# willow-ahrens/ChainPartitioners.jl

Measured on AMD Instinct MI355X. Metric: partitions/sec, DynamicTotalSplitter(AffineConnectivityModel{Int64}(0,0,0,1)), K=64, higher is better.
Workload: dtype int64; 1 GPU; config 3: DynamicTotalSplitter(AffineConnectivityModel{Int64}(0,0,0,1)) on suitesparse_shaped CSR (seeded SplitMix64 generator, tests/synth.py), n=10000000 rows, nnz=100000000, K=64; one independent partition per GPU; n=10000000, nnz=100000000, K=64, includes_oracle_build=True, device_block_pool=True

## Files before the change

### chainpartitioners.jl_amd/_lib.py

```python
from __future__ import annotations

import ctypes as C
import os
from functools import partial
import weakref

import numpy as np

from . import models as M

_HERE = os.path.dirname(os.path.abspath(__file__))
LIB_PATH = os.environ.get("CP_LIB_PATH") or os.path.join(_HERE, "libchainpart.so")


class _Array:

    def __init__(self, dtype, name):
        self.dtype, self.name, self.what = np.dtype(dtype), name, np.dtype(dtype).name

    def _accepts(self, a):
        return a.dtype == self.dtype

    def from_param(self, a):
        if a is None:
# ... 76 lines not shown
    "cp_dp_ptr_at": (_i32, [_vp, _i64, _i64, _pi64]),
    "cp_dp_ptr_row": (_i32, [_vp, _i64, _I64("out")]),
    "cp_dp_set_window": (_i32, [_vp, _i64]),
    "cp_dp_set_rows": (_i32, [_vp, _i64, _i64]),
    "cp_dp_block_tables": (_i32, [_vp, _pi32, _I64("opt_out"), _I64("nets_out"), _I64("selfnets_out")]),
    "cp_dp_destroy": (_i32, [_vp]),
    "cp_set_stream": (_i32, [_vp, _vp]),
    "cp_reset_stream": (_i32, [_vp]),
    "cp_get_stat": (_i32, [_str, _pi64]),
    "cp_test_round_scans": (_i32, [_I32("a"), _i64, _i64, _I32("b"), _i64, _i64, _i32, _i64, _i64, _i32, _i32,
                                   _I64("offs_out"), _I64("toffs_out"), _I64("res")]),
    "cp_test_fix_merge": (_i32, [_MODEL, _i64, _I64("toffs"), _I64("part_v"), _I32("part_p"), _I32("part_nn"), _I32("part_nl"), _I32("tile_s"),
                                 _I32("tile_s2"), _I32("anchor"), _I32("anchor2"), _I32("row"), _I32("plane"), _i64, _i32, _I32("p_out"),
                                 _I32("nn_out"), _I32("nl_out"), _I64("res")]),
    "cp_test_own_split": (_i32, [_vp, _I32("vpos_out"), _I32("vsa_out"), _I32("vnext_out"), _I64("res")]),
    "cp_set_option": (_i32, [_str, _i64]),
    "cp_prof_enable": (_i32, [_i32]),
    "cp_prof_reset": (_i32, []),
    "cp_prof_get": (_i32, [_i32, C.POINTER(C.c_char_p), _pi64, _pf64, _pf64]),
}
SYMBOLS = list(SIGNATURES)

_lib = None


def _typed(name, fn, restype, argtypes):
    fn.restype, fn.argtypes = restype, argtypes

    def call(*args):
        try:
# ... 129 lines not shown
        p, nn, res = np.zeros(ntask, np.int32), np.zeros(ntask, np.int32), np.zeros(4, np.int64)
        nl = None if part_nl is None else np.zeros(ntask, np.int32)
        rc = self.lib.cp_test_fix_merge(mm, ntask, toffs, part_v, i32(part_p), i32(part_nn), i32(part_nl), i32(tile_s), i32(tile_s2), i32(anchor),
                                        i32(anchor2), i32(row), i32(plane), n, reps, p, nn, nl, res)
        self._ok(rc, "cp_test_fix_merge")
        return p, nn, nl, dict(zip(("items", "trips", "edges", "tickets_left"), (int(v) for v in res)))

    def test_own_split(self, A):
        nb = max(0, int(A.n).bit_length() - 8)
        vpos = np.zeros((max(nb, 1), A.n + 1), np.int32); vsa = np.zeros_like(vpos)
        vnext = np.zeros(max(A.nnz, 1), np.int32); res = np.zeros(2, np.int64)
        rc = self.lib.cp_test_own_split(self._h(A), vpos.reshape(-1), vsa.reshape(-1), vnext, res)
        self._ok(rc, "cp_test_own_split")
        assert int(res[0]) == nb
        return nb, vpos[:nb], vsa[:nb], vnext[:int(res[1])]

    def set_option(self, name, value):
        return self.lib.cp_set_option(name.encode(), value)

    def partition_dynamic(self, A, K, combine, order, mm, rp, wm, wi, wf, spl):
        return self.lib.cp_partition_dynamic(self._h(A), K, combine, order, mm, rp, wm, wi, wf, spl)

    def pack_dynamic(self, A, mm, rp, wm, wi, wf, spl, Kout):
        return self.lib.cp_pack_dynamic(self._h(A), mm, rp, wm, wi, wf, spl, Kout)

    def pack_dynamic_tables(self, A, mm, rp, wm, wi, wf):
        spl = np.zeros(A.n + 1, dtype=np.int64)
        cst = _cost_zeros(mm, A.n + 1)
        rc = self.lib.cp_pack_dynamic_tables(self._h(A), mm, rp, wm, wi, wf, spl, *_by_type(cst))
        return rc, cst, spl
# ... 237 lines not shown
```

### chainpartitioners.jl_amd/csrc/capi.hip

```cpp
#include "csr.hpp"
#include "model.hpp"
#include "dp.hpp"
#include "weight.hpp"
#include "sym.hpp"
#include "cut.hpp"
#include <cmath>
#include <memory>

using namespace cpk;

namespace cpk {

__global__ void __launch_bounds__(256) k_range_counts(int64_t nq, const int64_t *__restrict__ P, const int64_t *__restrict__ Rr,
                                                      const int64_t *__restrict__ pos, const int32_t *__restrict__ prev,
                                                      const int64_t *__restrict__ fpos, const int32_t *__restrict__ flast,
                                                      unsigned long long *__restrict__ nets, unsigned long long *__restrict__ selfnets)
{
    int64_t i = blockIdx.x;
    if (i >= nq) return;
    __shared__ int64_t sh[256];
    int64_t p = P[i], r = Rr[i];
    int64_t stride = (int64_t)gridDim.y * 256, start = (int64_t)blockIdx.y * 256 + threadIdx.x;
    int64_t c = 0;
    if (r > p) {
// ... 94 lines not shown
static void also_f64(const int64_t *lo, const int64_t *hi, double *lo_f64, double *hi_f64) { *lo_f64 = (double)*lo; *hi_f64 = (double)*hi; }
static void also_f64(const double *, const double *, double *, double *) {}

template <typename TC>
static int32_t oracle_eval_into(cp_csr_t A, const cp_model_t *model, const cp_rowpart_t *Pi, int64_t nq, const int64_t *j, const int64_t *jp,
                                const int64_t *k, TC *out)
{
    const bool i64 = std::is_same<TC, int64_t>::value;
    return cp_oracle_eval(A, model, Pi, CP_HINT_STEP, nq, j, jp, k, i64 ? (int64_t *)out : nullptr, i64 ? nullptr : (double *)out);
}

static const struct { const char *name; int64_t *var; bool kept; } g_stats[] = {
    {"spec_redo", &g_spec_redo, false}, {"poison_hits", &g_poison_hits, false}, {"fix_trips", &g_fix_trips, false},
    {"fix_edges", &g_fix_edges, false}, {"fix_items", &g_fix_items, false}, {"bn_sym_layers", &g_bn_sym_layers, true},
    {"own_split_tiles", &g_own_split_tiles, false}, {"gap_split_tiles", &g_gap_split_tiles, false},
    {"overlap_isect", &g_overlap_isect, false}, {"cut_scan_layers", &g_cut_scan_layers, false},
};
static void stats_reset(bool all) { for (const auto &c : g_stats) if (all || !c.kept) *c.var = 0; }

enum OptRule { OPT_PLAIN, OPT_BOOL, OPT_CLAMP, OPT_POW2 };
constexpr int64_t NOLIM_LO = INT64_MIN, NOLIM_HI = INT64_MAX;
static const struct Opt { const char *name; int64_t *var; OptRule rule; int64_t lo, hi; } g_options[] = {
    {"force_brute", &g_opt_force_brute, OPT_PLAIN, 0, 0}, {"brute_max_n", &g_opt_brute_max_n, OPT_PLAIN, 0, 0}, {"dbg", &g_opt_dbg, OPT_PLAIN, 0, 0},
    {"short_t", &g_opt_short_t, OPT_PLAIN, 0, 0}, {"short_e", &g_opt_short_e, OPT_PLAIN, 0, 0}, {"ra_cache", &g_opt_ra_cache, OPT_PLAIN, 0, 0},
    {"leaf", &g_opt_leaf, OPT_PLAIN, 0, 0}, {"block_tables", &g_opt_block_tables, OPT_PLAIN, 0, 0}, {"nospec", &g_opt_nospec, OPT_PLAIN, 0, 0},
    {"rpass_small_tau", &g_opt_rpass_small_tau, OPT_PLAIN, 0, 0}, {"fixed_point", &g_opt_fixed_point, OPT_PLAIN, 0, 0},
    {"bn_wave", &g_opt_bn_wave, OPT_PLAIN, 0, 0},
    {"poison", &g_opt_poison, OPT_PLAIN, 0, 0},
    {"pool", &g_opt_pool, OPT_BOOL, 0, 0},
    {"own_blk", &g_opt_own_blk, OPT_BOOL, 0, 0},
    {"own_split", &g_opt_own_split, OPT_BOOL, 0, 0},
    {"gap_split", &g_opt_gap_split, OPT_BOOL, 0, 0},
    {"lws", &g_opt_lws, OPT_BOOL, 0, 0},
    {"gap_tau", &g_opt_gap_tau, OPT_CLAMP, NOLIM_LO, 20}, {"gap_min", &g_opt_gap_min, OPT_CLAMP, 8, NOLIM_HI}, {"gap_nr", &g_opt_gap_nr, OPT_CLAMP, 1, 2},
    {"force_max", &g_opt_force_max, OPT_CLAMP, 0, NOLIM_HI}, {"rpass_cap", &g_opt_rpass_cap, OPT_CLAMP, 1, NOLIM_HI},
    {"own_min", &g_opt_own_min, OPT_CLAMP, 64, NOLIM_HI}, {"bn_chunk", &g_opt_bn_chunk, OPT_CLAMP, 1, NOLIM_HI},
    {"bn_slack", &g_opt_bn_slack, OPT_CLAMP, 0, NOLIM_HI}, {"bn_run", &g_opt_bn_run, OPT_CLAMP, 2, NOLIM_HI},
    {"rpass_ch", &g_opt_rpass_ch, OPT_POW2, 16, 4096}, {"setup_bs", &g_opt_setup_bs, OPT_POW2, 64, 1024}, {"lws_leaf", &g_opt_lws_leaf, OPT_POW2, 256, 2048},
};
static int64_t opt_value(const Opt &o, int64_t value)
{
    switch (o.rule) {
    case OPT_BOOL: return value ? 1 : 0;
    case OPT_CLAMP: return value < o.lo ? o.lo : value > o.hi ? o.hi : value;
    case OPT_POW2: { int64_t v = o.lo; while (v < value && v < o.hi) v <<= 1; return v; }
    default: return value;
// ... 110 lines not shown
{
    if (!offs_out || !toffs_out || !res || (na > 0 && !a) || (nb > 0 && !b)) return CP_EINVAL;
    return guarded([&]() -> int32_t {
        dp_round_scans_test(a, na, na_max, b, nb, nb_max, two, cap_t, cap_nt, err_in, reps, offs_out, toffs_out, res);
        return CP_OK;
    });
}

int32_t cp_test_fix_merge(const cp_model_t *model, int64_t ntask, const int64_t *toffs, const int64_t *part_v, const int32_t *part_p, const int32_t *part_nn,
                          const int32_t *part_nl, const int32_t *tile_s, const int32_t *tile_s2, const int32_t *anchor, const int32_t *anchor2,
                          const int32_t *row, const int32_t *plane, int64_t n, int32_t reps, int32_t *p_out, int32_t *nn_out, int32_t *nl_out, int64_t *res)
{
    if (!model || !toffs || !part_v || !part_p || !part_nn || !tile_s || !anchor || !row || !plane || !p_out || !nn_out || !res) return CP_EINVAL;
    return guarded([&]() -> int32_t {
        dp_fix_merge_test(model, ntask, toffs, part_v, part_p, part_nn, part_nl, tile_s, tile_s2, anchor, anchor2, row, plane, n, reps, p_out, nn_out, nl_out, res);
        return CP_OK;
    });
}

int32_t cp_test_own_split(cp_csr_t A, int32_t *vpos_out, int32_t *vsa_out, int32_t *vnext_out, int64_t *res)
{
    if (!A || !vpos_out || !vsa_out || !vnext_out || !res) return CP_EINVAL;
    return guarded([&]() -> int32_t {
        CP_HIP(hipSetDevice(A->device));
        dp_own_split_test(A, vpos_out, vsa_out, vnext_out, res);
        return CP_OK;
    });
}

int32_t cp_reset_stream(cp_csr_t A)
// ... 440 lines not shown
```

### chainpartitioners.jl_amd/csrc/dp.hpp

```cpp
#pragma once
#include "csr.hpp"
#include "model.hpp"

struct cp_dp_s {
    cp_csr_s *A = nullptr;
    int64_t K = 0;
    int32_t combine = 0, order = 0;
    bool fast = false, fast_bn = false, need_self = false;
    void *work = nullptr;
    cpk::DBuf<int32_t> ptr;
    int64_t rlo = 0, rhi = 0;
    int64_t wwin = 0;
    std::vector<int64_t> lay_lo, lay_hi;
    virtual ~cp_dp_s() = default;
    virtual int32_t step_layer(int64_t k, const void *cst_prev_device, void *cst_cur_device) = 0;
    virtual int32_t block_tables(int32_t *nplanes_out, int64_t *opt_out, int64_t *nets_out, int64_t *selfnets_out) = 0;
};

namespace cpk {

using DpBase = ::cp_dp_s;

struct DpWindow {
    int64_t w = 0;
// ... 84 lines not shown
extern int64_t g_opt_ra_cache;
extern int64_t g_opt_fixed_point;
extern int64_t g_opt_nospec;
extern int64_t g_spec_redo;
extern int64_t g_opt_rpass_small_tau;
extern int64_t g_opt_force_max;
extern int64_t g_opt_setup_bs;
extern int64_t g_opt_rpass_cap;
extern int64_t g_opt_rpass_ch;
extern int64_t g_opt_own_min;
extern int64_t g_opt_own_blk;
extern int64_t g_opt_own_split;
extern int64_t g_own_split_tiles;
extern int64_t g_opt_gap_split;
extern int64_t g_gap_split_tiles;
extern int64_t g_overlap_isect;
void dp_own_split_test(cp_csr_s *A, int32_t *vpos_out, int32_t *vsa_out, int32_t *vnext_out, int64_t *res);
extern int64_t g_opt_short_t, g_opt_short_e;
extern int64_t g_opt_force_brute;
extern int64_t g_opt_brute_max_n;
extern int64_t g_opt_dbg;
enum DbgBit : int64_t {
    DBG_PRINT_ROUNDS = 8,
    DBG_NO_INTERIOR = 32,
    DBG_NO_OWN_TILES = 64,
    DBG_POISON = 128,
    DBG_POISON_ZERO = 256,
    DBG_GAP_ALL_SPECIAL = 512,
    DBG_MISPREDICT = 1024,
    DBG_TINY_BUFFERS = 2048,
// ... 14 lines not shown
```

### chainpartitioners.jl_amd/csrc/dp_brute.hip

```cpp
#include "csr.hpp"
#include "model.hpp"
#include "dp.hpp"

namespace cpk {

int64_t g_opt_force_brute = 0;
int64_t g_opt_short_t = 8, g_opt_short_e = 64;
int64_t g_opt_own_min = 64;
int64_t g_opt_own_blk = 1;
int64_t g_opt_own_split = 1;
int64_t g_own_split_tiles = 0;
int64_t g_opt_gap_split = 1;
int64_t g_gap_split_tiles = 0;
int64_t g_opt_rpass_ch = 256;
int64_t g_opt_rpass_small_tau = 4;
int64_t g_opt_force_max = 1024;
int64_t g_opt_setup_bs = 1024;
int64_t g_opt_rpass_cap = 200;
int64_t g_opt_nospec = 0, g_spec_redo = 0;
int64_t g_opt_gap_tau = 6, g_opt_gap_min = 64, g_opt_gap_nr = 2;
int64_t g_opt_ra_cache = 1;
int64_t g_opt_leaf = 1, g_opt_block_tables = 0;
int64_t g_opt_poison = 0, g_poison_hits = 0;
int64_t g_fix_trips = 0, g_fix_edges = 0, g_fix_items = 0;
int64_t g_opt_fixed_point = 0;
int64_t g_opt_brute_max_n = 200000;
int64_t g_opt_dbg = 0;

// ... 63 lines not shown
```

### chainpartitioners.jl_amd/csrc/dp_total.hip

```cpp
#include "dp_total.hpp"
#include <optional>

namespace cpk {

struct RoundDesc {
    int32_t isA, tau, nbits, nextra;
    Geo G;
    int64_t aoff[32];
    int64_t n, ntask;
    int64_t tbase[36];
    int64_t tskip[36];
    int64_t a_r0, a_nmain;
    int64_t extra[64];
    int32_t nlast, last_b[31];
    int32_t skip_std, skip_mir;
    int32_t fin_stamp;
};

__device__ __forceinline__ void decode_task(const RoundDesc &R, int64_t t, int64_t &r, int &b)
{
    if (R.G.win) {
        int bb = R.isA ? 0 : R.tau + 1;
        while (t >= R.tbase[bb + 1]) bb++;
        const int64_t l = t - R.tbase[bb] + R.tskip[bb];
// ... 640 lines not shown
                if (__ballot(inside)) {
                    int32_t cidx = inside ? idx : 0;
                    int src = cidx >> 2, comp = cidx & 3;
                    const int32_t g = __shfl(pack, src);
                    int32_t Fb = (g >> 3) + __popc((uint32_t)g & ((1u << comp) - 1u));
                    acc[k] += idx <= 0 ? tot : (inside ? tot - Fb : 0);
                } else {
                    acc[k] += idx <= 0 ? tot : 0;
                }
            }
        }
        c0 = n0; c1 = n1;
    }
}

__global__ void __launch_bounds__(256) k_own_map(RoundCounts *__restrict__ rc, const int64_t *__restrict__ toffs, const int4 *__restrict__ tdesc,
                                                 const int32_t *__restrict__ rlen, int4 *__restrict__ rec, int32_t *__restrict__ tile_task,
                                                 const uint8_t *__restrict__ tb, int32_t *__restrict__ gap_hi, int tau, int64_t n, int blk,
                                                 int32_t *__restrict__ bcnt, int32_t *__restrict__ brank, int2 *__restrict__ items,
                                                 int32_t *__restrict__ item_of, int split)
{
    const int64_t ntask = rc->nown, ntile = rc->NT;
    for (int64_t tile = (int64_t)blockIdx.x * blockDim.x + threadIdx.x; tile < ntile; tile += (int64_t)gridDim.x * blockDim.x) {
    int64_t lo = 0, hi = ntask;
    while (hi - lo > 1) {
        int64_t mid = (lo + hi) >> 1;
        if (toffs[mid] <= tile) lo = mid; else hi = mid;
    }
    int32_t kt = (int32_t)(tile - toffs[lo]);
    if (items) {
// ... 36 lines not shown
__global__ void __launch_bounds__(256) k_blk_order(const RoundCounts *__restrict__ rc, const int4 *__restrict__ rec, const int32_t *__restrict__ brank,
                                                   const int64_t *__restrict__ bstart, int32_t *__restrict__ border, int4 *__restrict__ srec,
                                                   int32_t *__restrict__ bcnt)
{
    const int64_t ntile = rc->NT;
    for (int64_t tile = (int64_t)blockIdx.x * blockDim.x + threadIdx.x; tile < ntile; tile += (int64_t)gridDim.x * blockDim.x) {
        const int4 r = rec[tile];
        const int32_t c = r.x / LT, rk = brank[tile];
        const int64_t slot = bstart[c] + rk;
        border[slot] = (int32_t)tile;
        srec[slot] = r;
        if (rk == 0) bcnt[c] = 0;
    }
}

template <typename TC, bool HYP, bool GAP>
__global__ void __launch_bounds__(256) k_lpass_own(int isA, const RoundCounts *__restrict__ rc, const int32_t *__restrict__ border,
                                                   const int32_t *__restrict__ a_pos, const int32_t *__restrict__ a_next,
                                                   const int32_t *__restrict__ a_fpos, const int32_t *__restrict__ a_flast,
                                                   int32_t *__restrict__ a_tileS, int32_t *__restrict__ a_tileS2, const int4 *__restrict__ a_rec,
                                                   const int4 *__restrict__ a_srec, const TC *__restrict__ W, DevModel<TC> M, TC alpha, Best<TC, HYP> *__restrict__ part,
                                                   int tau, const int32_t *__restrict__ gap_hi, uint8_t *__restrict__ spec, int force_spec,
                                                   Best<TC, HYP> *__restrict__ sub, int32_t *__restrict__ spv,
                                                   const int32_t *__restrict__ a_col, const int32_t *__restrict__ a_ffirst,
                                                   const int32_t *__restrict__ a_vnext, const int32_t *__restrict__ a_vpos,
                                                   const int32_t *__restrict__ a_vsa, int64_t vstride)
{
    int lane = threadIdx.x & 63;
    int64_t tile = (int64_t)blockIdx.x * 4 + __builtin_amdgcn_readfirstlane(threadIdx.x >> 6);
    if (tile >= rc->NT) return;
    const int4 vrec = border ? a_srec[tile] : a_rec[tile];
    if (border) tile = border[tile];
    const int32_t rw = __builtin_amdgcn_readfirstlane(vrec.w);
    const int4 rec = make_int4(__builtin_amdgcn_readfirstlane(vrec.x), __builtin_amdgcn_readfirstlane(vrec.y), __builtin_amdgcn_readfirstlane(vrec.z), rw);
    int head = rw & 1;
    int32_t tl = (rw >> 2) & 255;
    int32_t acc[4], acc2[4] = {0, 0, 0, 0}, sk[4], sk2[4];
    __shared__ int32_t s_es_all[4][2][SMAX + 1], s_v_all[4][2][SMAX + 1];
    __shared__ int32_t s_cnt_all[4];
    int32_t(*s_es)[SMAX + 1] = s_es_all[threadIdx.x >> 6], (*s_v)[SMAX + 1] = s_v_all[threadIdx.x >> 6];
    int ns = 0;
    if (GAP && (rw & 2)) {
        int32_t *s_cnt = &s_cnt_all[threadIdx.x >> 6];
// ... 1523 lines not shown
        const unsigned grid = (unsigned)cdiv(n1, 256);
        hipLaunchKernelGGL(k_split_count, dim3(grid), dim3(256), 0, s, A->pos32.p, A->next.p, n, S.nb, S.vsa.p);
        exclusive_scan_i32_i32(S.vsa.p, S.vpos.p, (int64_t)cells, scratch, s);
        hipLaunchKernelGGL(k_split_scatter, dim3(grid), dim3(256), 0, s, A->pos32.p, A->next.p, n, S.nb, S.vpos.p, S.vnext.p, S.vsa.p);
        CP_HIP(hipGetLastError());
        int32_t st[SPLIT_NB + 1];
        for (int b = 0; b <= S.nb; b++)
            CP_HIP(hipMemcpyAsync(&st[b], S.vpos.p + (size_t)b * (size_t)n1, sizeof(int32_t), hipMemcpyDeviceToHost, s));
        CP_HIP(hipStreamSynchronize(s));
        for (int b = 0; b < S.nb; b++) S.tot[b] = (int64_t)st[b + 1] - st[b];
        S.tot[S.nb] = st[S.nb];
    }
    S.built = true;
}

void dp_own_split_test(cp_csr_s *A, int32_t *vpos_out, int32_t *vsa_out, int32_t *vnext_out, int64_t *res)
{
    ensure_links(A);
    SplitLinks S;
    DBuf<int64_t> scratch;
    split_build(A, S, scratch);
    res[0] = S.nb; res[1] = S.tot[S.nb];
    if (S.nb <= 0) return;
    const size_t cells = (size_t)S.nb * (size_t)S.stride;
    CP_HIP(hipMemcpyAsync(vpos_out, S.vpos.p, cells * sizeof(int32_t), hipMemcpyDeviceToHost, A->stream));
    CP_HIP(hipMemcpyAsync(vsa_out, S.vsa.p, cells * sizeof(int32_t), hipMemcpyDeviceToHost, A->stream));
    if (res[1] > 0) CP_HIP(hipMemcpyAsync(vnext_out, S.vnext.p, (size_t)res[1] * sizeof(int32_t), hipMemcpyDeviceToHost, A->stream));
    CP_HIP(hipStreamSynchronize(A->stream));
}

// ... 365 lines not shown
{
    hipStream_t s = C.s;
    ProfScope ps(PROF_SCAN, s, 12.0 * (double)R.ntask);
    const bool tiny = C.spec && (g_opt_dbg & DBG_TINY_BUFFERS);
    const int64_t capT = C.spec ? (tiny ? (int64_t)64 : (int64_t)Wk.fl.loc.n) : INT64_MAX, capNT = C.spec ? (tiny ? (int64_t)1 : (int64_t)Wk.ow.o_rec.n) : INT64_MAX;
    const int64_t nm = std::min<int64_t>(R.ntask, (int64_t)Wk.ow.o_ntl.n);
    if (R.ntask <= LB_MAX) {
        launch_round_scans(rc, Wk.tk.len.p, Wk.tk.offs.p, R.ntask, Wk.ow.o_ntl.p, Wk.ow.o_toffs.p, nm, C.own_tiles, capT, capNT, Wk.sc.scanws, s);
    } else {
        exclusive_scan_i32_devn(Wk.tk.len.p, Wk.tk.offs.p, &rc->nlong, R.ntask, &rc->T, Wk.sc.scratch, s);
        if (C.own_tiles) exclusive_scan_i32_devn(Wk.ow.o_ntl.p, Wk.ow.o_toffs.p, &rc->nown, nm, &rc->NT, Wk.sc.scratch, s);
        hipLaunchKernelGGL(k_round_finish, dim3(1), dim3(1), 0, s, rc, capT, capNT);
    }
}

template <typename TC, bool HYP>
static void own_stream(const LayerCtx<TC> &C, LayerWork<TC> &Wk, const RoundDesc &R, RoundCounts *rc, const RoundCounts &P, bool gap, int split)
{
    hipStream_t s = C.s;
    cp_csr_s *A = C.A;
    const int64_t n = C.n;
    const int oblk = C.oblk;
    const int64_t gNT = C.spec ? (int64_t)Wk.ow.o_rec.n : P.NT;
    poison_fill(s, {{Wk.ow.o_part.p, Wk.ow.o_part.bytes()}, {Wk.ow.o_tileS.p, Wk.ow.o_tileS.bytes()}, {Wk.ow.o_rec.p, Wk.ow.o_rec.bytes()}, {Wk.ow.o_srec.p, Wk.ow.o_srec.bytes()},
                    {if_hyp<HYP>(Wk.ow.o_tileS2.p), Wk.ow.o_tileS2.bytes()}, {Wk.ow.o_items.p, Wk.ow.o_items.bytes()}, {Wk.ow.o_item_of.p, Wk.ow.o_item_of.bytes()},
                    {Wk.ow.o_trec.p, Wk.ow.o_trec.bytes()}});
    const unsigned mgrid = (unsigned)std::min<int64_t>(cdiv(gNT, 256), 8192);
    if (split && !Wk.ow.split.built) {
        ProfScope ps(PROF_LINKS, s, 8.0 * (double)A->N + 16.0 * (double)(C.nbits - SPLIT_BMIN) * (double)(n + 1));
        split_build(A, Wk.ow.split, Wk.sc.scratch);
    }
    hipLaunchKernelGGL(k_own_map, dim3(mgrid), dim3(256), 0, s, rc, Wk.ow.o_toffs.p, Wk.ow.o_tdesc.p, Wk.ow.o_rlen.p, Wk.ow.o_rec.p, Wk.ow.o_task.p,
                       Wk.ow.o_tb.p, gap ? Wk.ow.o_hi.p : (int32_t *)nullptr, R.tau, n, oblk, oblk ? Wk.ow.b_cnt.p : (int32_t *)nullptr, Wk.ow.o_brank.p,
                       gap ? (int2 *)nullptr : Wk.ow.o_items.p, Wk.ow.o_item_of.p, split);
    ProfScope ps(gap ? PROF_GAPSTREAM : PROF_OWN, s, C.own_bytes(Wk.ow.split, R.tau, split != 0, (double)P.own_steps));
    if (oblk) {
        exclusive_scan_i32_lb(Wk.ow.b_cnt.p, Wk.ow.b_start.p, Wk.ow.b_n.p, Wk.ow.b_nblk, nullptr, Wk.sc.scanws, s);
        hipLaunchKernelGGL(k_blk_order, dim3(mgrid), dim3(256), 0, s, rc, Wk.ow.o_rec.p, Wk.ow.o_brank.p, Wk.ow.b_start.p, Wk.ow.o_border.p, Wk.ow.o_srec.p, Wk.ow.b_cnt.p);
    }
    hipLaunchKernelGGL(HIP_KERNEL_NAME(gap ? k_lpass_own<TC, HYP, true> : k_lpass_own<TC, HYP, false>), dim3((unsigned)cdiv(gNT, 4)), dim3(256), 0, s,
                       R.isA, rc,
                       oblk ? Wk.ow.o_border.p : (const int32_t *)nullptr, A->pos32.p, A->next.p, if_hyp<HYP>(A->fpos32.p), if_hyp<HYP>(A->flast.p),
                       Wk.ow.o_tileS.p, Wk.ow.o_tileS2.p, Wk.ow.o_rec.p, Wk.ow.o_srec.p, C.W, C.M, C.alpha, recs<HYP>(Wk.ow.o_part), R.tau, Wk.ow.o_hi.p, Wk.ow.o_spec.p,
                       (int)((g_opt_dbg & DBG_GAP_ALL_SPECIAL) != 0), recs<HYP>(Wk.ow.o_sub), Wk.ow.o_spv.p, A->col.p, if_hyp<HYP>(A->ffirst.p),
                       split ? Wk.ow.split.vnext.p : (const int32_t *)nullptr, Wk.ow.split.vpos.p, Wk.ow.split.vsa.p, (int64_t)(n + 1));
}

template <typename TC, bool HYP>
static void own_merge(const LayerCtx<TC> &C, LayerWork<TC> &Wk, RoundCounts *rc, const RoundCounts &P)
{
    ProfScope ps(PROF_FIX, C.s, 24.0 * (double)P.NT);
    launch_fix_own<TC, HYP>(C.s, rc, Wk.ow.o_toffs.p, recs<HYP>(Wk.ow.o_part), Wk.ow.o_tdesc.p, Wk.ow.o_tb.p, if_hyp<HYP>(Wk.ow.o_tS0l.p), Wk.ow.o_tileS.p,
                            if_hyp<HYP>(Wk.ow.o_tileS2.p), C.M, Wk.pl.opt.p, Wk.pl.nnopt.p, if_hyp<HYP>(Wk.pl.nlopt.p), C.n, Wk.ow.o_items.p, Wk.ow.o_item_of.p, Wk.ow.o_trec.p,
                            Wk.ow.o_tick.p, C.spec ? grow_pred(P.NT) : P.NT, C.spec ? grow_pred(P.nown) : P.nown);
}

// ... 125 lines not shown
    hipStream_t s = C.s;
    const int64_t n = C.n;
    const Geo G = C.G;
    const int nbits = C.nbits;
    int32_t *pzp = C.pzp;
    const int NR = nbits + 1;
    std::vector<RoundCounts> used((size_t)NR);
    memset(used.data(), 0, sizeof(RoundCounts) * (size_t)NR);
    struct Patch { size_t idx; int rd; int kind; int tau; bool split; };
    std::vector<Patch> patches;
    auto note = [&](int rd, int kind, int slot, int tau = 0, bool sp = false) {
        if (prof_active(slot)) patches.push_back({g_prof_pending.size() - 1, rd, kind, tau, sp});
    };
    bool any_forced = false;
    std::vector<int8_t> split_mode((size_t)NR, 0);

    for (int rd = 0; rd <= nbits; rd++) {
        RoundDesc R;
        if (rd == 0) make_round(R, true, 0, nbits, n, rlo, rhi, G, Wk.win.aoff);
        else make_round(R, false, nbits - rd, nbits, n, rlo, rhi, G, Wk.win.aoff);
        R.fin_stamp = Wk.pl.fin_stamp;
        if (C.leaf && !R.isA && R.tau < LEAF_T) continue;
        if (rd == 0 && g_opt_ra_cache && rlo <= 1 && rhi >= n && n >= 1 && !G.win) {
            round_a_full<TC, HYP>(C, Wk);
            R.a_nmain = 0; R.ntask = R.nextra + R.nlast;
        }
        if (rd == 0 && g_opt_ra_cache && G.win && G.s >= 1 && n >= 1 && !(g_opt_dbg & DBG_WIN_NO_RA_CACHE)) {
            std::optional<ProfScope> scope;
            round_a_win_std<TC, HYP>(C, Wk, scope);
            R.skip_std = 1;
// ... 22 lines not shown
            Wk.fl.ensure_flat(Wk.hyp, (size_t)grow_pred(P.T));
        }
        round_scans<TC>(C, Wk, R, rc);
        if (!spec) {
            CP_HIP(hipMemcpyAsync(&P, rc, sizeof(P), hipMemcpyDeviceToHost, s));
            CP_HIP(hipStreamSynchronize(s));
            Wk.ow.ensure_own(Wk.hyp, (size_t)P.NT);
            Wk.fl.ensure_flat(Wk.hyp, (size_t)P.T);
        }
        used[(size_t)rd] = P;
        if (g_opt_dbg & DBG_PRINT_ROUNDS) fprintf(stderr, "round isA=%d tau=%d ntask=%lld %s long=%d own=%d T=%lld NT=%lld nontrivial=%d\n", R.isA, R.tau, (long long)R.ntask,
                                   spec ? "predicted" : "exact", P.nlong, P.nown, (long long)P.T, (long long)P.NT, P._pad);
        if (P.nown > 0 && P.NT > 0) {
            const int split = !(C.split_layer && !R.isA && (!gap || g_opt_gap_split)) ? 0 : R.tau + 1 >= SPLIT_BMIN ? 1 : 2;
            split_mode[(size_t)rd] = (int8_t)(gap ? -split : split);
            own_stream<TC, HYP>(C, Wk, R, rc, P, gap, split);
            note(rd, 0, gap ? PROF_GAPSTREAM : PROF_OWN, R.tau, split != 0);
            if (gap) gap_finish<TC, HYP>(C, Wk, R, rc, P);
            else own_merge<TC, HYP>(C, Wk, rc, P);
            CP_HIP(hipGetLastError());
        }
        if (P.nlong <= 0 || P.T <= 0) continue;
        flat_stream<TC, HYP>(C, Wk, R, rc, P);
        note(rd, 1, PROF_EXPAND);
        flat_finish<TC, HYP>(C, Wk, R, rc, P);
    }
    if (C.leaf) leaf_pass<TC, HYP>(C, Wk);
    combine_rows<TC, HYP>(C, Wk);
    CP_HIP(hipGetLastError());
    std::vector<RoundCounts> got((size_t)NR);
// ... 9 lines not shown
        if (g.nown > 0 && g.NT > 0 && !(u.nown > 0 && u.NT > 0)) ok = false;
        if (g.nlong > 0 && g.T > 0 && !(u.nlong > 0 && u.T > 0)) ok = false;
    }
    if (pzp) {
        g_poison_hits += pz_hits[0];
        CP_REQUIRE(!(ok && pz_hits[0] > 0), CP_EINTERNAL, "a DP layer that is not redone read plane cells nobody wrote (poison mode)");
    }
    if (ok) Wk.ow.b_dirty = false;
    Wk.ow.t_dirty = false;
    if (ok) for (int rd = 0; rd < NR; rd++) { g_fix_trips += got[(size_t)rd].n_trips; g_fix_edges |= got[(size_t)rd].n_edge; }
    if (ok) for (int rd = 0; rd < NR; rd++) {
        const RoundCounts &g = got[(size_t)rd];
        if (g.nown > 0 && g.NT > 0) {
            const int sm = split_mode[(size_t)rd];
            (sm < 0 ? g_gap_split_tiles : g_own_split_tiles) += std::abs(sm) == 1 ? g.NT : std::abs(sm) == 2 ? g.n_split : 0;
        }
    }
    for (int rd = 0; rd < NR; rd++) g_fix_items += got[(size_t)rd].n_items;
    if (ok) {
        for (auto &pt : patches) {
            const RoundCounts &g = got[(size_t)pt.rd];
            if (pt.idx < g_prof_pending.size())
                g_prof_pending[pt.idx].bytes = pt.kind == 0 ? C.own_bytes(Wk.ow.split, pt.tau, pt.split, (double)g.own_steps) : (double)g.T * C.step_bytes;
        }
        Wk.sp.pred = got; Wk.sp.pred_ok = true; Wk.sp.pred_rlo = rlo; Wk.sp.pred_rhi = rhi; Wk.sp.pred_win = G.win; Wk.sp.pred_w = G.w;
        if (allow_force && 2 * (rhi - rlo + 1) >= Wk.sp.force_rows) {
            Wk.sp.force_own.resize((size_t)NR, 0);
            Wk.sp.force_rows = rhi - rlo + 1;
            for (int rd = 1; rd < NR; rd++) {
                const RoundCounts &g = got[(size_t)rd];
// ... 118 lines not shown
```

### include/chainpart.h

```cpp
#ifndef CHAINPART_H
#define CHAINPART_H

#include "chainpart_types.h"

#ifdef __cplusplus
extern "C" {
#endif

typedef struct cp_csr_s *cp_csr_t;
typedef struct cp_count_s *cp_count_t;

const char *cp_last_error(void);
int32_t cp_version(void);
int32_t cp_device_count(void);

int32_t cp_csr_create(int64_t m, int64_t n, int64_t N, const int64_t *colptr, const int64_t *rowval,
                      int32_t device, cp_csr_t *out);
int32_t cp_csr_create_device(int64_t m, int64_t n, int64_t N, const int64_t *colptr_device,
                             const int64_t *rowval_device, int32_t device, cp_csr_t *out);
int32_t cp_csr_destroy(cp_csr_t csr);
int32_t cp_adjoint(cp_csr_t csr, cp_csr_t *out);
int32_t cp_csr_download(cp_csr_t csr, int64_t *dims_out, int64_t *colptr_out, int64_t *rowval_out);
int32_t cp_csr_reset_cache(cp_csr_t csr);

// ... 96 lines not shown
int32_t cp_dp_set_window(cp_dp_t dp, int64_t wmax);
int32_t cp_dp_set_rows(cp_dp_t dp, int64_t row_lo, int64_t row_hi);
int32_t cp_dp_block_tables(cp_dp_t dp, int32_t *nplanes_out, int64_t *opt_out, int64_t *nets_out, int64_t *selfnets_out);
int32_t cp_dp_destroy(cp_dp_t dp);

int32_t cp_set_stream(cp_csr_t csr, void *hip_stream);
int32_t cp_reset_stream(cp_csr_t csr);
int32_t cp_get_stat(const char *name, int64_t *out);
int32_t cp_test_round_scans(const int32_t *a, int64_t na, int64_t na_max, const int32_t *b, int64_t nb, int64_t nb_max, int32_t two,
                            int64_t cap_t, int64_t cap_nt, int32_t err_in, int32_t reps, int64_t *offs_out, int64_t *toffs_out, int64_t *res);
int32_t cp_test_fix_merge(const cp_model_t *model, int64_t ntask, const int64_t *toffs, const int64_t *part_v, const int32_t *part_p,
                          const int32_t *part_nn, const int32_t *part_nl, const int32_t *tile_s, const int32_t *tile_s2, const int32_t *anchor,
                          const int32_t *anchor2, const int32_t *row, const int32_t *plane, int64_t n, int32_t reps, int32_t *p_out,
                          int32_t *nn_out, int32_t *nl_out, int64_t *res);
int32_t cp_test_own_split(cp_csr_t csr, int32_t *vpos_out, int32_t *vsa_out, int32_t *vnext_out, int64_t *res);
int32_t cp_set_option(const char *name, int64_t value);
int32_t cp_prof_enable(int32_t on);
int32_t cp_prof_reset(void);
int32_t cp_prof_get(int32_t slot, const char **name, int64_t *launches, double *total_ms, double *alg_bytes);

#ifdef __cplusplus
}
#endif
#endif
```

Baseline: 2.652 partitions/s.

## Process two own-stream tiles per wavefront with interleaved loads

Adds a paired mode to the own-pass kernel in which each wavefront handles two tiles. The second tile's head and first data loads are issued while the first tile's stream is being processed, which hides memory latency. Each wave does twice the work and the grid is half as large. The mode is on by default for the non-hypergraph, non-gap, non-window case. It brings extra register pressure, lower wave parallelism, and serialized tail work for odd tile counts.

After: 2.704 partitions/s, median of 6. 1.02x the previous value.

```diff
diff --git a/chainpartitioners.jl_amd/_lib.py b/chainpartitioners.jl_amd/_lib.py
--- a/chainpartitioners.jl_amd/_lib.py
+++ b/chainpartitioners.jl_amd/_lib.py
@@ -114,6 +114,7 @@
                                  _I32("tile_s2"), _I32("anchor"), _I32("anchor2"), _I32("row"), _I32("plane"), _i64, _i32, _I32("p_out"),
                                  _I32("nn_out"), _I32("nl_out"), _I64("res")]),
     "cp_test_own_split": (_i32, [_vp, _I32("vpos_out"), _I32("vsa_out"), _I32("vnext_out"), _I64("res")]),
+    "cp_test_own_pair": (_i32, [_i64, _i64, _I64("res")]),
     "cp_set_option": (_i32, [_str, _i64]),
     "cp_prof_enable": (_i32, [_i32]),
     "cp_prof_reset": (_i32, []),
@@ -273,6 +274,11 @@
         self._ok(rc, "cp_test_own_split")
         assert int(res[0]) == nb
         return nb, vpos[:nb], vsa[:nb], vnext[:int(res[1])]
+
+    def test_own_pair(self, nt, wave):
+        res = np.zeros(3, np.int64)
+        self._ok(self.lib.cp_test_own_pair(nt, wave, res), "cp_test_own_pair")
+        return bool(res[0]), int(res[1]), int(res[2])
 
     def set_option(self, name, value):
         return self.lib.cp_set_option(name.encode(), value)
diff --git a/chainpartitioners.jl_amd/csrc/capi.hip b/chainpartitioners.jl_amd/csrc/capi.hip
--- a/chainpartitioners.jl_amd/csrc/capi.hip
+++ b/chainpartitioners.jl_amd/csrc/capi.hip
@@ -132,6 +132,7 @@
     {"spec_redo", &g_spec_redo, false}, {"poison_hits", &g_poison_hits, false}, {"fix_trips", &g_fix_trips, false},
     {"fix_edges", &g_fix_edges, false}, {"fix_items", &g_fix_items, false}, {"bn_sym_layers", &g_bn_sym_layers, true},
     {"own_split_tiles", &g_own_split_tiles, false}, {"gap_split_tiles", &g_gap_split_tiles, false},
+    {"own_pair_waves", &g_own_pair_waves, false}, {"own_pair_lone", &g_own_pair_lone, false},
     {"overlap_isect", &g_overlap_isect, false}, {"cut_scan_layers", &g_cut_scan_layers, false},
 };
 static void stats_reset(bool all) { for (const auto &c : g_stats) if (all || !c.kept) *c.var = 0; }
@@ -148,6 +149,7 @@
     {"pool", &g_opt_pool, OPT_BOOL, 0, 0},
     {"own_blk", &g_opt_own_blk, OPT_BOOL, 0, 0},
     {"own_split", &g_opt_own_split, OPT_BOOL, 0, 0},
+    {"own_pair", &g_opt_own_pair, OPT_BOOL, 0, 0},
     {"gap_split", &g_opt_gap_split, OPT_BOOL, 0, 0},
     {"lws", &g_opt_lws, OPT_BOOL, 0, 0},
     {"gap_tau", &g_opt_gap_tau, OPT_CLAMP, NOLIM_LO, 20}, {"gap_min", &g_opt_gap_min, OPT_CLAMP, 8, NOLIM_HI}, {"gap_nr", &g_opt_gap_nr, OPT_CLAMP, 1, 2},
@@ -288,6 +290,15 @@
     if (!model || !toffs || !part_v || !part_p || !part_nn || !tile_s || !anchor || !row || !plane || !p_out || !nn_out || !res) return CP_EINVAL;
     return guarded([&]() -> int32_t {
         dp_fix_merge_test(model, ntask, toffs, part_v, part_p, part_nn, part_nl, tile_s, tile_s2, anchor, anchor2, row, plane, n, reps, p_out, nn_out, nl_out, res);
+        return CP_OK;
+    });
+}
+
+int32_t cp_test_own_pair(int64_t nt, int64_t wave, int64_t *res)
+{
+    if (!res) return CP_EINVAL;
+    return guarded([&]() -> int32_t {
+        dp_own_pair_test(nt, wave, res);
         return CP_OK;
     });
 }
diff --git a/chainpartitioners.jl_amd/csrc/dp.hpp b/chainpartitioners.jl_amd/csrc/dp.hpp
--- a/chainpartitioners.jl_amd/csrc/dp.hpp
+++ b/chainpartitioners.jl_amd/csrc/dp.hpp
@@ -122,6 +122,9 @@
 extern int64_t g_own_split_tiles;
 extern int64_t g_opt_gap_split;
 extern int64_t g_gap_split_tiles;
+extern int64_t g_opt_own_pair;
+extern int64_t g_own_pair_waves, g_own_pair_lone;
+void dp_own_pair_test(int64_t nt, int64_t wave, int64_t *res);
 extern int64_t g_overlap_isect;
 void dp_own_split_test(cp_csr_s *A, int32_t *vpos_out, int32_t *vsa_out, int32_t *vnext_out, int64_t *res);
 extern int64_t g_opt_short_t, g_opt_short_e;
diff --git a/chainpartitioners.jl_amd/csrc/dp_brute.hip b/chainpartitioners.jl_amd/csrc/dp_brute.hip
--- a/chainpartitioners.jl_amd/csrc/dp_brute.hip
+++ b/chainpartitioners.jl_amd/csrc/dp_brute.hip
@@ -12,6 +12,8 @@
 int64_t g_own_split_tiles = 0;
 int64_t g_opt_gap_split = 1;
 int64_t g_gap_split_tiles = 0;
+int64_t g_opt_own_pair = 1;
+int64_t g_own_pair_waves = 0, g_own_pair_lone = 0;
 int64_t g_opt_rpass_ch = 256;
 int64_t g_opt_rpass_small_tau = 4;
 int64_t g_opt_force_max = 1024;
diff --git a/chainpartitioners.jl_amd/csrc/dp_total.hip b/chainpartitioners.jl_amd/csrc/dp_total.hip
--- a/chainpartitioners.jl_amd/csrc/dp_total.hip
+++ b/chainpartitioners.jl_amd/csrc/dp_total.hip
@@ -678,6 +678,120 @@
     }
 }
 
+struct TileHead { int32_t cp[4], pv[4], ptop, qhi, qlo; };
+struct TileRun { int32_t Q_lo, Q_hi, x, x_end; int4 c0, c1; };
+
+__device__ __forceinline__ void tile_head_loads(TileHead &h, const int32_t *__restrict__ cpos, const int32_t *__restrict__ psum, int32_t p_first, int32_t tl,
+                                                int head, int lane)
+{
+    const int32_t *__restrict__ cl = cpos + (p_first - tl), *__restrict__ pl = (psum ? psum : cpos) + (p_first - tl);
+#pragma unroll
+    for (int k = 0; k < 4; k++) {
+        const int32_t e = lane + 64 * k;
+        const uint32_t d = (uint32_t)(tl - (e < tl ? e : tl)) & 255u;
+        h.cp[k] = cl[d];
+        h.pv[k] = pl[d];
+    }
+    h.ptop = pl[tl + 1 - head];
+    h.qhi = cl[tl + 1 - head];
+    h.qlo = cl[0];
+}
+
+__device__ __forceinline__ int4 tile_quad(const int32_t *__restrict__ arr, int32_t x, int32_t x_end, uint32_t o)
+{
+    const uint32_t r = (uint32_t)(x_end - x);
+    return *reinterpret_cast<const int4 *>(arr + x + (o < r ? o : r));
+}
+
+__device__ __forceinline__ void tile_counters(const TileHead &h, int32_t tl, int lane, bool psum, int32_t acc[4], int32_t sk[4], TileRun &r)
+{
+    r.Q_hi = __builtin_amdgcn_readfirstlane(h.qhi);
+    r.Q_lo = __builtin_amdgcn_readfirstlane(h.qlo);
+#pragma unroll
+    for (int k = 0; k < 4; k++) {
+        const bool on = lane + 64 * k <= tl;
+        sk[k] = on ? h.cp[k] : INT32_MAX;
+        acc[k] = (psum && on) ? h.ptop - h.pv[k] : 0;
+    }
+    r.x_end = r.Q_hi & ~3;
+    r.x = r.Q_lo & ~3;
+}
+
+__device__ __forceinline__ void tile_first(const int32_t *__restrict__ arr, int lane, TileRun &r)
+{
+    r.c0 = tile_quad(arr, r.x, r.x_end, 4 * lane);
+    r.c1 = tile_quad(arr, r.x, r.x_end, 256 + 4 * lane);
+}
+
+template <bool GE, bool DET = false>
+__device__ __forceinline__ void tile_trips(const int32_t *__restrict__ arr, TileRun &r, int32_t thr, int lane, int32_t acc[4], const int32_t sk[4],
+                                           int32_t sp_lo = 0, int32_t sp_hi = 0, int32_t *s_es = nullptr, int32_t *s_v = nullptr, int32_t *s_cnt = nullptr,
+                                           int kind = 0)
+{
+    const int32_t Q_lo = r.Q_lo, Q_hi = r.Q_hi, x_end = r.x_end;
+    int32_t x = r.x;
+    int4 c0 = r.c0, c1 = r.c1;
+    for (; x < Q_hi; x += 512) {
+        const int4 n0 = tile_quad(arr, x, x_end, 512 + 4 * lane), n1 = tile_quad(arr, x, x_end, 768 + 4 * lane);
+#pragma unroll
+        for (int c = 0; c < 2; c++) {
+            int32_t xc = x + c * 256;
+            if (xc >= Q_hi) break;
+            int4 v = c ? c1 : c0;
+            int32_t pb = xc + 4 * lane;
+            const bool inner = xc >= Q_lo && xc + 256 <= Q_hi;
+            bool f0 = GE ? v.x >= thr : v.x < thr, f1 = GE ? v.y >= thr : v.y < thr, f2 = GE ? v.z >= thr : v.z < thr, f3 = GE ? v.w >= thr : v.w < thr;
+            if (!inner) { f0 = f0 && pb < Q_hi; f1 = f1 && pb + 1 < Q_hi; f2 = f2 && pb + 2 < Q_hi; f3 = f3 && pb + 3 < Q_hi; }
+            const unsigned long long m0 = __ballot(f0), m1 = __ballot(f1), m2 = __ballot(f2), m3 = __ballot(f3);
+            if (DET) {
+                const uint32_t span = (uint32_t)(sp_hi - sp_lo - 1);
+                bool s0 = (uint32_t)(v.x - sp_lo - 1) < span, s1 = (uint32_t)(v.y - sp_lo - 1) < span, s2 = (uint32_t)(v.z - sp_lo - 1) < span,
+                     s3 = (uint32_t)(v.w - sp_lo - 1) < span;
+                if (!inner) {
+                    s0 = s0 && pb >= Q_lo && pb < Q_hi; s1 = s1 && pb + 1 >= Q_lo && pb + 1 < Q_hi;
+                    s2 = s2 && pb + 2 >= Q_lo && pb + 2 < Q_hi; s3 = s3 && pb + 3 >= Q_lo && pb + 3 < Q_hi;
+                }
+                if (s0 || s1 || s2 || s3) {
+#pragma unroll
+                    for (int j = 0; j < 4; j++) {
+                        if (j == 0 ? s0 : j == 1 ? s1 : j == 2 ? s2 : s3) {
+                            int32_t val = j == 0 ? v.x : j == 1 ? v.y : j == 2 ? v.z : v.w;
+                            int slot = atomicAdd(s_cnt, 1);
+                            if (slot <= SMAX - 1) {
+                                s_es[slot] = pb + j;
+                                s_v[slot] = (int32_t)(((uint32_t)val & 0x7fffffffu) | ((uint32_t)kind << 31));
+                            }
+                        }
+                    }
+                }
+            }
+            int32_t tot = __popcll(m0) + __popcll(m1) + __popcll(m2) + __popcll(m3);
+            uint32_t P0 = 0;
+            P0 = __builtin_amdgcn_mbcnt_hi((uint32_t)(m0 >> 32), __builtin_amdgcn_mbcnt_lo((uint32_t)m0, P0));
+            P0 = __builtin_amdgcn_mbcnt_hi((uint32_t)(m1 >> 32), __builtin_amdgcn_mbcnt_lo((uint32_t)m1, P0));
+            P0 = __builtin_amdgcn_mbcnt_hi((uint32_t)(m2 >> 32), __builtin_amdgcn_mbcnt_lo((uint32_t)m2, P0));
+            P0 = __builtin_amdgcn_mbcnt_hi((uint32_t)(m3 >> 32), __builtin_amdgcn_mbcnt_lo((uint32_t)m3, P0));
+            const int32_t pack = (int32_t)((P0 << 3) | (uint32_t)f0 | ((uint32_t)f1 << 1) | ((uint32_t)f2 << 2));
+#pragma unroll
+            for (int k = 0; k < 4; k++) {
+                int32_t idx = sk[k] - xc;
+                bool inside = idx > 0 && idx < 256;
+                if (__ballot(inside)) {
+                    int32_t cidx = inside ? idx : 0;
+                    int src = cidx >> 2, comp = cidx & 3;
+                    const int32_t g = __shfl(pack, src);
+                    int32_t Fb = (g >> 3) + __popc((uint32_t)g & ((1u << comp) - 1u));
+                    acc[k] += idx <= 0 ? tot : (inside ? tot - Fb : 0);
+                } else {
+                    acc[k] += idx <= 0 ? tot : 0;
+                }
+            }
+        }
+        c0 = n0; c1 = n1;
+    }
+}
+
+
 __global__ void __launch_bounds__(256) k_own_map(RoundCounts *__restrict__ rc, const int64_t *__restrict__ toffs, const int4 *__restrict__ tdesc,
                                                  const int32_t *__restrict__ rlen, int4 *__restrict__ rec, int32_t *__restrict__ tile_task,
                                                  const uint8_t *__restrict__ tb, int32_t *__restrict__ gap_hi, int tau, int64_t n, int blk,
@@ -744,7 +858,46 @@
     }
 }
 
-template <typename TC, bool HYP, bool GAP>
+template <typename TC, bool HYP>
+__device__ __forceinline__ void own_tile_cands(Best<TC, HYP> cand[4], const int4 rec, int32_t tl, int head, int isA, const DevModel<TC> &M, TC alpha, int lane,
+                                               const int32_t acc[4], const int32_t acc2[4], const int32_t sk[4], const TC wv[4])
+{
+#pragma unroll
+    for (int k = 0; k < 4; k++) {
+        int32_t e = lane + 64 * k;
+        best_clear(cand[k]);
+        if (e <= tl && !(head && isA && e == 0)) {
+            int32_t p = rec.x - e;
+            TC fv = dm_apply_affine(M, alpha, (int64_t)(rec.y - p), (int64_t)(rec.z - sk[k]), (int64_t)acc[k], (int64_t)acc2[k]);
+            cand[k].v = cadd(wv[k], fv); cand[k].p = p; cand[k].nn = acc[k]; best_set_nl(cand[k], acc2[k]);
+        }
+    }
+}
+
+template <typename TC, bool HYP>
+__device__ __forceinline__ Best<TC, HYP> own_tile_winner(const Best<TC, HYP> cand[4], int lane)
+{
+    Best<TC, HYP> best; best_clear(best);
+#pragma unroll
+    for (int k = 0; k < 4; k++) best = better(best, cand[k]);
+    for (int o = 32; o > 0; o >>= 1) {
+        int src = (lane + o) & 63;
+        Best<TC, HYP> c; best_clear(c); c.v = shfl64(best.v, src); c.p = __shfl(best.p, src); c.nn = __shfl(best.nn, src);
+        if (HYP) best_set_nl(c, __shfl(best_nl(best), src));
+        bool take = (best.p < 0) ? (c.p >= 0) : (c.p >= 0 && (c.v < best.v || (c.v == best.v && c.p > best.p)));
+        if (lane + o < 64 && take) best = c;
+    }
+    return best;
+}
+
+__host__ __device__ __forceinline__ bool own_pair_slots(int64_t w, int64_t nt, int64_t &s0, int64_t &s1)
+{
+    s0 = 2 * w;
+    s1 = 2 * w + 1 < nt ? 2 * w + 1 : s0;
+    return w >= 0 && s0 < nt;
+}
+
+template <typename TC, bool HYP, bool GAP, bool PAIR = false>
 __global__ void __launch_bounds__(256) k_lpass_own(int isA, const RoundCounts *__restrict__ rc, const int32_t *__restrict__ border,
                                                    const int32_t *__restrict__ a_pos, const int32_t *__restrict__ a_next,
                                                    const int32_t *__restrict__ a_fpos, const int32_t *__restrict__ a_flast,
@@ -757,6 +910,66 @@
                                                    const int32_t *__restrict__ a_vsa, int64_t vstride)
 {
     int lane = threadIdx.x & 63;
+    if constexpr (PAIR && !HYP && !GAP) {
+        int64_t s0, s1;
+        if (!own_pair_slots((int64_t)blockIdx.x * 4 + __builtin_amdgcn_readfirstlane(threadIdx.x >> 6), rc->NT, s0, s1)) return;
+        const bool lone = s1 == s0;
+        const uint32_t pinm = M.p[CP_P_PIN] != (TC)0 ? 255u : 0u;
+        const int4 vA = border ? a_srec[s0] : a_rec[s0], vB = border ? a_srec[s1] : a_rec[s1];
+        int64_t tA = s0, tB = s1;
+        if (border) { tA = border[s0]; tB = border[s1]; }
+        const int4 rA = make_int4(__builtin_amdgcn_readfirstlane(vA.x), __builtin_amdgcn_readfirstlane(vA.y), __builtin_amdgcn_readfirstlane(vA.z),
+                                  __builtin_amdgcn_readfirstlane(vA.w));
+        const int4 rB = make_int4(__builtin_amdgcn_readfirstlane(vB.x), __builtin_amdgcn_readfirstlane(vB.y), __builtin_amdgcn_readfirstlane(vB.z),
+                                  __builtin_amdgcn_readfirstlane(vB.w));
+        const int hdA = rA.w & 1, hdB = rB.w & 1;
+        const int32_t tlA = (rA.w >> 2) & 255, tlB = (rB.w >> 2) & 255;
+        const int sbA = rA.w >> 10, sbB = rB.w >> 10;
+        const int64_t soA = sbA ? (int64_t)(sbA - SPLIT_BMIN) * vstride : 0, soB = sbB ? (int64_t)(sbB - SPLIT_BMIN) * vstride : 0;
+        const int32_t *__restrict__ arrA = sbA ? a_vnext : a_next, *__restrict__ arrB = sbB ? a_vnext : a_next;
+        TileHead hB;
+        tile_head_loads(hB, sbB ? a_vpos + soB : a_pos, sbB ? a_vsa + soB : (const int32_t *)nullptr, rB.x, tlB, hdB, lane);
+        TileRun uB;
+        int32_t accA[4], accB[4], skA[4], skB[4];
+        const int32_t zero4[4] = {0, 0, 0, 0};
+        interior_stream<true>(arrA, sbA ? a_vpos + soA : a_pos, rA.x, tlA, rA.y, lane, accA, skA, hdA, 0, 0, nullptr, nullptr, nullptr, 0,
+                              sbA ? a_vsa + soA : (const int32_t *)nullptr);
+        tile_counters(hB, tlB, lane, sbB != 0, accB, skB, uB);
+        TC wv[4];
+#pragma unroll
+        for (int k = 0; k < 4; k++) {
+            const int32_t e = lane + 64 * k;
+            const uint32_t d = (uint32_t)(tlA - (e < tlA ? e : tlA)) & 255u;
+            skA[k] = (a_pos + (rA.x - tlA))[d & pinm];
+            wv[k] = (W + (rA.x - tlA))[d];
+        }
+        tile_first(arrB, lane, uB);
+        Best<TC, HYP> cand[4];
+        {
+            const int sel = tlA >> 6;
+            if (lane == (tlA & 63)) a_tileS[tA] = sel == 0 ? accA[0] : sel == 1 ? accA[1] : sel == 2 ? accA[2] : accA[3];
+            own_tile_cands<TC, HYP>(cand, rA, tlA, hdA, isA, M, alpha, lane, accA, zero4, skA, wv);
+            const Best<TC, HYP> best = own_tile_winner<TC, HYP>(cand, lane);
+            if (lane == 0) part[tA] = best;
+        }
+        tile_trips<true>(arrB, uB, rB.y, lane, accB, skB);
+#pragma unroll
+        for (int k = 0; k < 4; k++) {
+            const int32_t e = lane + 64 * k;
+            const uint32_t d = (uint32_t)(tlB - (e < tlB ? e : tlB)) & 255u;
+            skB[k] = (a_pos + (rB.x - tlB))[d & pinm];
+            wv[k] = (W + (rB.x - tlB))[d];
+        }
+        if (lone) return;
+        {
+            const int sel = tlB >> 6;
+            if (lane == (tlB & 63)) a_tileS[tB] = sel == 0 ? accB[0] : sel == 1 ? accB[1] : sel == 2 ? accB[2] : accB[3];
+            own_tile_cands<TC, HYP>(cand, rB, tlB, hdB, isA, M, alpha, lane, accB, zero4, skB, wv);
+            const Best<TC, HYP> best = own_tile_winner<TC, HYP>(cand, lane);
+            if (lane == 0) part[tB] = best;
+        }
+        return;
+    }
     int64_t tile = (int64_t)blockIdx.x * 4 + __builtin_amdgcn_readfirstlane(threadIdx.x >> 6);
     if (tile >= rc->NT) return;
     const int4 vrec = border ? a_srec[tile] : a_rec[tile];
@@ -2310,6 +2523,14 @@
     S.built = true;
 }
 
+void dp_own_pair_test(int64_t nt, int64_t wave, int64_t *res)
+{
+    int64_t s0 = 0, s1 = 0;
+    res[0] = own_pair_slots(wave, nt, s0, s1) ? 1 : 0;
+    res[1] = s0;
+    res[2] = s1;
+}
+
 void dp_own_split_test(cp_csr_s *A, int32_t *vpos_out, int32_t *vsa_out, int32_t *vnext_out, int64_t *res)
 {
     ensure_links(A);
@@ -2705,6 +2926,8 @@
     }
 }
 
+template <bool HYP> static bool own_pairs(bool gap, bool win) { return !HYP && !gap && !win && g_opt_own_pair != 0; }
+
 template <typename TC, bool HYP>
 static void own_stream(const LayerCtx<TC> &C, LayerWork<TC> &Wk, const RoundDesc &R, RoundCounts *rc, const RoundCounts &P, bool gap, int split)
 {
@@ -2729,8 +2952,9 @@
         exclusive_scan_i32_lb(Wk.ow.b_cnt.p, Wk.ow.b_start.p, Wk.ow.b_n.p, Wk.ow.b_nblk, nullptr, Wk.sc.scanws, s);
         hipLaunchKernelGGL(k_blk_order, dim3(mgrid), dim3(256), 0, s, rc, Wk.ow.o_rec.p, Wk.ow.o_brank.p, Wk.ow.b_start.p, Wk.ow.o_border.p, Wk.ow.o_srec.p, Wk.ow.b_cnt.p);
     }
-    hipLaunchKernelGGL(HIP_KERNEL_NAME(gap ? k_lpass_own<TC, HYP, true> : k_lpass_own<TC, HYP, false>), dim3((unsigned)cdiv(gNT, 4)), dim3(256), 0, s,
-                       R.isA, rc,
+    const bool pair = own_pairs<HYP>(gap, C.G.win != 0);
+    hipLaunchKernelGGL(HIP_KERNEL_NAME(gap ? k_lpass_own<TC, HYP, true> : pair ? k_lpass_own<TC, HYP, false, !HYP> : k_lpass_own<TC, HYP, false>),
+                       dim3((unsigned)cdiv(pair ? cdiv(gNT, 2) : gNT, 4)), dim3(256), 0, s, R.isA, rc,
                        oblk ? Wk.ow.o_border.p : (const int32_t *)nullptr, A->pos32.p, A->next.p, if_hyp<HYP>(A->fpos32.p), if_hyp<HYP>(A->flast.p),
                        Wk.ow.o_tileS.p, Wk.ow.o_tileS2.p, Wk.ow.o_rec.p, Wk.ow.o_srec.p, C.W, C.M, C.alpha, recs<HYP>(Wk.ow.o_part), R.tau, Wk.ow.o_hi.p, Wk.ow.o_spec.p,
                        (int)((g_opt_dbg & DBG_GAP_ALL_SPECIAL) != 0), recs<HYP>(Wk.ow.o_sub), Wk.ow.o_spv.p, A->col.p, if_hyp<HYP>(A->ffirst.p),
@@ -2886,6 +3110,7 @@
     };
     bool any_forced = false;
     std::vector<int8_t> split_mode((size_t)NR, 0);
+    std::vector<int8_t> pair_mode((size_t)NR, 0);
 
     for (int rd = 0; rd <= nbits; rd++) {
         RoundDesc R;
@@ -2938,6 +3163,7 @@
         if (P.nown > 0 && P.NT > 0) {
             const int split = !(C.split_layer && !R.isA && (!gap || g_opt_gap_split)) ? 0 : R.tau + 1 >= SPLIT_BMIN ? 1 : 2;
             split_mode[(size_t)rd] = (int8_t)(gap ? -split : split);
+            pair_mode[(size_t)rd] = own_pairs<HYP>(gap, G.win != 0);
             own_stream<TC, HYP>(C, Wk, R, rc, P, gap, split);
             note(rd, 0, gap ? PROF_GAPSTREAM : PROF_OWN, R.tau, split != 0);
             if (gap) gap_finish<TC, HYP>(C, Wk, R, rc, P);
@@ -2977,6 +3203,7 @@
         if (g.nown > 0 && g.NT > 0) {
             const int sm = split_mode[(size_t)rd];
             (sm < 0 ? g_gap_split_tiles : g_own_split_tiles) += std::abs(sm) == 1 ? g.NT : std::abs(sm) == 2 ? g.n_split : 0;
+            if (pair_mode[(size_t)rd]) { g_own_pair_waves += g.NT / 2; g_own_pair_lone += g.NT & 1; }
         }
     }
     for (int rd = 0; rd < NR; rd++) g_fix_items += got[(size_t)rd].n_items;
diff --git a/include/chainpart.h b/include/chainpart.h
--- a/include/chainpart.h
+++ b/include/chainpart.h
@@ -134,6 +134,7 @@
                           const int32_t *anchor2, const int32_t *row, const int32_t *plane, int64_t n, int32_t reps, int32_t *p_out,
                           int32_t *nn_out, int32_t *nl_out, int64_t *res);
 int32_t cp_test_own_split(cp_csr_t csr, int32_t *vpos_out, int32_t *vsa_out, int32_t *vnext_out, int64_t *res);
+int32_t cp_test_own_pair(int64_t nt, int64_t wave, int64_t *res);
 int32_t cp_set_option(const char *name, int64_t value);
 int32_t cp_prof_enable(int32_t on);
 int32_t cp_prof_reset(void);
```
